# cswhjiang/Recurrent_Fusion_Network

Hardware: AMD Instinct MI355X
Metric: captions/sec (train fwd+bwd) at B=256, M=4, L=196, D=2048, seq=16; 1/2/4/8 GPU (higher is better)
Workload: dtype f32; 1 GPU; C3: RecurrentFusionModel XE train step (zero_grad+fwd+criterion+bwd+clamp+Adam), M=4 encoders, L=196, D=2048, R=A=E=512, T1=T2=8, K=1000, V+1=9488, seq=16 (17 decoder steps); captions_per_gpu=256, global_batch=256, parallelism=single GPU, micro_batches=1, updates=51, hip_graph=False, overlap_update=False, fused_loss=False, gemm_flags=0

## Files before the change

### recurrent_fusion_network_amd/csrc/rfn_adam.hip

```cpp
#include <string.h>

#include "rfn_common.h"

typedef float f32x4 __attribute__((ext_vector_type(4)));

__device__ __forceinline__ void adam_elem(float& pv, float gv, float& mv, float& vv, float lr_over_bc1, float beta1,
                                          float beta2, float eps, float inv_sqrt_bc2, float wd, float clip,
                                          float gscale) {
#pragma clang fp contract(off)
    gv *= gscale;
    gv = fminf(fmaxf(gv, -clip), clip);
    gv = __builtin_fmaf(wd, pv, gv);
    mv = __builtin_fmaf(beta1, mv, (1.0f - beta1) * gv);
    vv = __builtin_fmaf(beta2, vv, ((1.0f - beta2) * gv) * gv);
    pv = pv - (lr_over_bc1 * mv) / __builtin_fmaf(sqrtf(vv), inv_sqrt_bc2, eps);
}
struct AdamBuckets {
    float* p[RFN_ADAM_MAXBUCKET];
    const float* g[RFN_ADAM_MAXBUCKET];
    float* m[RFN_ADAM_MAXBUCKET];
    float* v[RFN_ADAM_MAXBUCKET];
    long n[RFN_ADAM_MAXBUCKET];
    int vec[RFN_ADAM_MAXBUCKET];
    int nb;
};
__global__ __launch_bounds__(256) void adam_multi_k(const AdamBuckets B, float lr_over_bc1, float beta1, float beta2, float eps,
                                                    float inv_sqrt_bc2, float wd, float clip, float gscale,
                                                    const float* __restrict__ coef) {
    if (coef) {
        lr_over_bc1 = coef[0];
        inv_sqrt_bc2 = coef[1];
    }
    const long stride = (long)gridDim.x * 256, i0 = (long)blockIdx.x * 256 + threadIdx.x;
    for (int k = 0; k < B.nb; ++k) {
        if (B.vec[k]) {
            const long n4 = B.n[k] >> 2;
            f32x4* p4 = reinterpret_cast<f32x4*>(B.p[k]);
            const f32x4* g4 = reinterpret_cast<const f32x4*>(B.g[k]);
            f32x4* m4 = reinterpret_cast<f32x4*>(B.m[k]);
            f32x4* v4 = reinterpret_cast<f32x4*>(B.v[k]);
            for (long i = i0; i < n4; i += stride) {
                f32x4 pv = p4[i], mv = m4[i], vv = v4[i];
                const f32x4 gv = g4[i];
#pragma unroll
                for (int e = 0; e < 4; ++e) {
                    float pe = pv[e], me = mv[e], ve = vv[e];
                    adam_elem(pe, gv[e], me, ve, lr_over_bc1, beta1, beta2, eps, inv_sqrt_bc2, wd, clip, gscale);
                    pv[e] = pe;
                    mv[e] = me;
                    vv[e] = ve;
                }
                m4[i] = mv;
                v4[i] = vv;
                p4[i] = pv;
            }
        } else {
            float* p = B.p[k];
            const float* g = B.g[k];
            float* m = B.m[k];
            float* v = B.v[k];
            for (long i = i0; i < B.n[k]; i += stride) {
                float pv = p[i], mv = m[i], vv = v[i];
                adam_elem(pv, g[i], mv, vv, lr_over_bc1, beta1, beta2, eps, inv_sqrt_bc2, wd, clip, gscale);
                m[i] = mv;
                v[i] = vv;
                p[i] = pv;
            }
        }
    }
}
static int adam_multi_launch(int nbuckets, float* const* p, const float* const* g, float* const* m, float* const* v,
                             const int64_t* n, float lr, float beta1, float beta2, float eps, float weight_decay,
                             float grad_clip, float grad_scale, int step, const float* coef, void* stream) {
    if (nbuckets < 1 || nbuckets > RFN_ADAM_MAXBUCKET || (!coef && step < 1)) return RFN_ERR_SHAPE;
    if (!p || !g || !m || !v || !n) return RFN_ERR_ARG;
    AdamBuckets B;
    memset(&B, 0, sizeof(B));
    long most = 0;
    for (int k = 0; k < nbuckets; ++k) {
        if (n[k] <= 0) return RFN_ERR_SHAPE;
        if (!p[k] || !g[k] || !m[k] || !v[k]) return RFN_ERR_ARG;
        B.p[k] = p[k]; B.g[k] = g[k]; B.m[k] = m[k]; B.v[k] = v[k]; B.n[k] = (long)n[k];
        B.vec[k] = (n[k] % 4 == 0) && rfn_aligned16(p[k]) && rfn_aligned16(g[k]) && rfn_aligned16(m[k]) && rfn_aligned16(v[k]);
        const long work = B.vec[k] ? (long)n[k] / 4 : (long)n[k];
        most = work > most ? work : most;
    }
    B.nb = nbuckets;
    float c0 = 0.f, c1 = 0.f;
    if (!coef) {
        const double bc1 = 1.0 - pow((double)beta1, step), bc2 = 1.0 - pow((double)beta2, step);
        c0 = (float)(lr / bc1);
        c1 = (float)(1.0 / sqrt(bc2));
    }
    const int blocks = (int)(most / 256 + 1 < 4096 ? most / 256 + 1 : 4096);
    hipLaunchKernelGGL(adam_multi_k, dim3(blocks), dim3(256), 0, (hipStream_t)stream, B, c0, beta1, beta2, eps, c1, weight_decay,
                       grad_clip, grad_scale, coef);
    RFN_CHECK_LAUNCH();
    return RFN_OK;
}
extern "C" int rfn_adam_step_multi(int nbuckets, float* const* p, const float* const* g, float* const* m, float* const* v,
                                   const int64_t* n, float lr, float beta1, float beta2, float eps, float weight_decay,
                                   float grad_clip, float grad_scale, int step, void* stream) {
    return adam_multi_launch(nbuckets, p, g, m, v, n, lr, beta1, beta2, eps, weight_decay, grad_clip, grad_scale, step, nullptr,
                             stream);
}
extern "C" int rfn_adam_step_multi_coef(int nbuckets, float* const* p, const float* const* g, float* const* m, float* const* v,
                                        const int64_t* n, const float* coef_dev, float beta1, float beta2, float eps,
                                        float weight_decay, float grad_clip, float grad_scale, void* stream) {
    if (!coef_dev) return RFN_ERR_ARG;
    return adam_multi_launch(nbuckets, p, g, m, v, n, 0.f, beta1, beta2, eps, weight_decay, grad_clip, grad_scale, 0, coef_dev,
                             stream);
}
extern "C" int rfn_adam_step(float* p, const float* g, float* m, float* v, int64_t n, float lr, float beta1,
                             float beta2, float eps, float weight_decay, float grad_clip, float grad_scale, int step,
                             void* stream) {
    return adam_multi_launch(1, &p, &g, &m, &v, &n, lr, beta1, beta2, eps, weight_decay, grad_clip, grad_scale, step, nullptr,
                             stream);
}
```

Measured before the change: 3985 captions/s.

## Flatten Adam buckets into contiguous spans with occupancy-sized grid and nontemporal loads

The multi-bucket Adam kernel now splits every vectorised bucket into fixed-size spans indexed through a prefix table. Blocks grid-stride over the global span list, so each block streams a contiguous chunk instead of striding across all buckets in turn. The grid is capped at resident blocks (occupancy times CU count) instead of a fixed 4096. Loads and stores of m, v and g use nontemporal hints to avoid polluting cache. This targets DRAM streaming efficiency and launch tail, at the cost of a per-span bucket lookup and possible load imbalance when the span count is small.

Measured after the change: 4001 captions/s, median of 6. About the same (+0.4%).

```diff
diff --git a/recurrent_fusion_network_amd/csrc/rfn_adam.hip b/recurrent_fusion_network_amd/csrc/rfn_adam.hip
--- a/recurrent_fusion_network_amd/csrc/rfn_adam.hip
+++ b/recurrent_fusion_network_amd/csrc/rfn_adam.hip
@@ -15,15 +15,28 @@
     vv = __builtin_fmaf(beta2, vv, ((1.0f - beta2) * gv) * gv);
     pv = pv - (lr_over_bc1 * mv) / __builtin_fmaf(sqrtf(vv), inv_sqrt_bc2, eps);
 }
+#ifndef ADAM_SPAN4
+#define ADAM_SPAN4 1024
+#endif
+#ifndef ADAM_NT
+#define ADAM_NT 1
+#endif
+static_assert(ADAM_SPAN4 % 256 == 0, "a span is a whole number of block trips");
 struct AdamBuckets {
     float* p[RFN_ADAM_MAXBUCKET];
     const float* g[RFN_ADAM_MAXBUCKET];
     float* m[RFN_ADAM_MAXBUCKET];
     float* v[RFN_ADAM_MAXBUCKET];
     long n[RFN_ADAM_MAXBUCKET];
+    long span0[RFN_ADAM_MAXBUCKET + 1];
     int vec[RFN_ADAM_MAXBUCKET];
     int nb;
 };
+__device__ __forceinline__ f32x4 adam_ld(const f32x4* a) { return ADAM_NT ? __builtin_nontemporal_load(a) : *a; }
+__device__ __forceinline__ void adam_st(f32x4* a, const f32x4& x) {
+    if (ADAM_NT) __builtin_nontemporal_store(x, a);
+    else *a = x;
+}
 __global__ __launch_bounds__(256) void adam_multi_k(const AdamBuckets B, float lr_over_bc1, float beta1, float beta2, float eps,
                                                     float inv_sqrt_bc2, float wd, float clip, float gscale,
                                                     const float* __restrict__ coef) {
@@ -31,30 +44,34 @@
         lr_over_bc1 = coef[0];
         inv_sqrt_bc2 = coef[1];
     }
+    const long nspan = B.span0[B.nb];
+    int k = 0;
+    for (long w = blockIdx.x; w < nspan; w += gridDim.x) {
+        while (w >= B.span0[k + 1]) ++k;
+        const long n4 = B.n[k] >> 2, s0 = (w - B.span0[k]) * ADAM_SPAN4, s1 = s0 + ADAM_SPAN4 < n4 ? s0 + ADAM_SPAN4 : n4;
+        f32x4* p4 = reinterpret_cast<f32x4*>(B.p[k]);
+        const f32x4* g4 = reinterpret_cast<const f32x4*>(B.g[k]);
+        f32x4* m4 = reinterpret_cast<f32x4*>(B.m[k]);
+        f32x4* v4 = reinterpret_cast<f32x4*>(B.v[k]);
+        for (long i = s0 + threadIdx.x; i < s1; i += 256) {
+            f32x4 pv = p4[i], mv = adam_ld(m4 + i), vv = adam_ld(v4 + i);
+            const f32x4 gv = adam_ld(g4 + i);
+#pragma unroll
+            for (int e = 0; e < 4; ++e) {
+                float pe = pv[e], me = mv[e], ve = vv[e];
+                adam_elem(pe, gv[e], me, ve, lr_over_bc1, beta1, beta2, eps, inv_sqrt_bc2, wd, clip, gscale);
+                pv[e] = pe;
+                mv[e] = me;
+                vv[e] = ve;
+            }
+            adam_st(m4 + i, mv);
+            adam_st(v4 + i, vv);
+            p4[i] = pv;
+        }
+    }
     const long stride = (long)gridDim.x * 256, i0 = (long)blockIdx.x * 256 + threadIdx.x;
     for (int k = 0; k < B.nb; ++k) {
-        if (B.vec[k]) {
-            const long n4 = B.n[k] >> 2;
-            f32x4* p4 = reinterpret_cast<f32x4*>(B.p[k]);
-            const f32x4* g4 = reinterpret_cast<const f32x4*>(B.g[k]);
-            f32x4* m4 = reinterpret_cast<f32x4*>(B.m[k]);
-            f32x4* v4 = reinterpret_cast<f32x4*>(B.v[k]);
-            for (long i = i0; i < n4; i += stride) {
-                f32x4 pv = p4[i], mv = m4[i], vv = v4[i];
-                const f32x4 gv = g4[i];
-#pragma unroll
-                for (int e = 0; e < 4; ++e) {
-                    float pe = pv[e], me = mv[e], ve = vv[e];
-                    adam_elem(pe, gv[e], me, ve, lr_over_bc1, beta1, beta2, eps, inv_sqrt_bc2, wd, clip, gscale);
-                    pv[e] = pe;
-                    mv[e] = me;
-                    vv[e] = ve;
-                }
-                m4[i] = mv;
-                v4[i] = vv;
-                p4[i] = pv;
-            }
-        } else {
+        if (!B.vec[k]) {
             float* p = B.p[k];
             const float* g = B.g[k];
             float* m = B.m[k];
@@ -69,6 +86,19 @@
         }
     }
 }
+static long adam_resident_blocks() {
+    static long slots[16] = {};
+    int dev = 0;
+    hipGetDevice(&dev);
+    long& s = slots[dev & 15];
+    if (s == 0) {
+        int occ = 0, cus = 256;
+        if (hipOccupancyMaxActiveBlocksPerMultiprocessor(&occ, adam_multi_k, 256, 0) != hipSuccess || occ < 1) occ = 1;
+        if (hipDeviceGetAttribute(&cus, hipDeviceAttributeMultiprocessorCount, dev) != hipSuccess || cus < 1) cus = 256;
+        s = (long)occ * cus;
+    }
+    return s;
+}
 static int adam_multi_launch(int nbuckets, float* const* p, const float* const* g, float* const* m, float* const* v,
                              const int64_t* n, float lr, float beta1, float beta2, float eps, float weight_decay,
                              float grad_clip, float grad_scale, int step, const float* coef, void* stream) {
@@ -82,7 +112,8 @@
         if (!p[k] || !g[k] || !m[k] || !v[k]) return RFN_ERR_ARG;
         B.p[k] = p[k]; B.g[k] = g[k]; B.m[k] = m[k]; B.v[k] = v[k]; B.n[k] = (long)n[k];
         B.vec[k] = (n[k] % 4 == 0) && rfn_aligned16(p[k]) && rfn_aligned16(g[k]) && rfn_aligned16(m[k]) && rfn_aligned16(v[k]);
-        const long work = B.vec[k] ? (long)n[k] / 4 : (long)n[k];
+        B.span0[k + 1] = B.span0[k] + (B.vec[k] ? ((long)n[k] / 4 + ADAM_SPAN4 - 1) / ADAM_SPAN4 : 0);
+        const long work = B.vec[k] ? B.span0[k + 1] : (long)n[k] / 256 + 1;
         most = work > most ? work : most;
     }
     B.nb = nbuckets;
@@ -92,7 +123,8 @@
         c0 = (float)(lr / bc1);
         c1 = (float)(1.0 / sqrt(bc2));
     }
-    const int blocks = (int)(most / 256 + 1 < 4096 ? most / 256 + 1 : 4096);
+    const long cap = adam_resident_blocks();
+    const int blocks = (int)(most < cap ? most : cap);
     hipLaunchKernelGGL(adam_multi_k, dim3(blocks), dim3(256), 0, (hipStream_t)stream, B, c0, beta1, beta2, eps, c1, weight_decay,
                        grad_clip, grad_scale, coef);
     RFN_CHECK_LAUNCH();
```
